# bridgedp/hunter_bipedal_control

Hardware: NVIDIA H100
Metric: MPC+WBC control-step solves/sec (Hunter N=100) (higher is better)
Workload: dtype f64

## Files before the change

hunter_bipedal_control_b200/csrc/hb_sqp.cuh:

```cuda
#pragma once
#include "hb_common.cuh"
#include "hb_mpc.cuh"
#include "hb_planner.h"
#include "hb_rbd.cuh"

namespace hb {

constexpr int LIN_F1 = 0, LIN_F2 = 22, LIN_A1 = 44, LIN_A2 = 242, LIN_BF1 = 440, LIN_BF2 = 476, LIN_BV1 = 512, LIN_BV2 = 572,
              LIN_EPOS = 632, LIN_EVEL = 644, LIN_DPQ = 656, LIN_DVX = 812, LIN_DVV = 1076, LIN_STRIDE = 1200;
constexpr int NTMAX = 16;
constexpr int NVMAX = 8;
constexpr int PJ_BT = 0, PJ_AT = 144, PJ_PXV = 342, PJ_NV = 562, PJ_BTV = 642, PJ_QV = 664, PJ_RV = 686, PJ_META = 702, PJ_PEV = 710,
              PJ_QT = 720, PJ_PT = 1204, PJ_RF = 1380, PJ_RN = 1416, PJ_STRIDE = 1480;
constexpr int PJ_RT_PACKED = PJ_STRIDE - PJ_RF;
static_assert(PJ_AT + 9 * NX == PJ_PXV && PJ_RN + NVMAX * NVMAX == PJ_STRIDE && PJ_PEV + NJ == PJ_QT, "projected record blocks are contiguous");
static_assert(PJ_QT % 2 == 0 && PJ_PT % 2 == 0 && PJ_RF % 2 == 0 && PJ_STRIDE % 2 == 0, "bulk-copied blocks start on 16 bytes");
constexpr int RK_STRIDE = NTMAX * NX + NTMAX;

struct LinHalf {
  double x[NX], u[NU], x2[NX], f[NX];
  double Acm[6 * 16], Jc[12 * 16], dp[12 * NDIR], dv[12 * NDIR];
  double Abinv[36], AbinvAj[6 * NJ], vgen[16], epos[12], evel[12], com[3];
  double sn[NDIR], cs[NDIR];
  double dh[6 * NDIR], dcom[3 * NDIR], dvb[6 * NDIR];
  double vals[2 * 6];
};
static_assert(16 * 9 <= 6 * NDIR + 3 * NDIR + 6 * NDIR, "partial sums must fit in the dh | dcom | dvb storage");

__device__ __noinline__ void lin_half(LinHalf& sh, const ChainModel& cm, const double* xs, int hl, bool act, double* rec_f, double* rec_A, double* rec_Bf,
                                      double* rec_Bv, bool want_ee, double* rec) {
  const double m = c_model.total_mass, im = 1.0 / m;
  double* part = sh.dh;
  if (hl < NDIR) { double s, c; sincos(xs[9 + hl], &s, &c); sh.sn[hl] = s; sh.cs[hl] = c; }
  __syncwarp();
  const bool euler = hl < 6;
  const int leg = (hl < 3 || (hl >= 6 && hl < 11)) ? 0 : 1;
  const int gen = euler ? 3 + (hl % 3) : hl;
  const bool with_base = hl < 3;
  const bool vlane = (hl == 0 || hl == 3);
  {
    ChainOut<double> co;
    kin_chain_f<double>(cm, leg, with_base, [&](int i) { return xs[6 + i]; }, [&](int i) { return (i == gen) ? 1.0 : 0.0; },
                        [&](int k, double& s, double& c) { s = sh.sn[k]; c = sh.cs[k]; }, co);
#pragma unroll
    for (int i = 0; i < 3; ++i) { part[hl * 9 + i] = co.P[i]; part[hl * 9 + 3 + i] = co.Lo[i]; }
    if (vlane) {
#pragma unroll
      for (int i = 0; i < 3; ++i) sh.vals[(hl / 3) * 6 + 3 + i] = co.mc[i];
    }
#pragma unroll
    for (int t = 0; t < 2; ++t) {
      const int c = leg + 2 * t;
#pragma unroll
      for (int i = 0; i < 3; ++i) {
        sh.Jc[(3 * c + i) * 16 + gen] = co.cvel[3 * t + i];
        if (!euler) sh.Jc[(3 * (c ^ 1) + i) * 16 + gen] = 0.0;
        if (vlane) sh.epos[3 * c + i] = co.cpos[3 * t + i];
      }
    }
    if (hl < 3) {
#pragma unroll
      for (int r = 0; r < 6; ++r) sh.Acm[r * 16 + hl] = (r == hl) ? m : 0.0;
#pragma unroll
// ... 41 lines not shown
  }
  if (hl >= 6) sh.vgen[hl] = sh.u[6 + hl];
  __syncwarp();
  if (hl < NJ) {
#pragma unroll
    for (int r = 0; r < 6; ++r) { double s = 0.0; for (int c = 0; c < 6; ++c) s += sh.Abinv[6 * r + c] * sh.Acm[c * 16 + 6 + hl]; sh.AbinvAj[r * NJ + hl] = s; }
  }
  {
    const int dir = gen - 3;
    ChainOut<D1> co;
    kin_chain_f<D1>(cm, leg, with_base, [&](int i) { return D1(xs[6 + i], (i == gen) ? 1.0 : 0.0); }, [&](int i) { return D1(sh.vgen[i], 0.0); },
                    [&](int k, D1& s, D1& c) { const double sv = sh.sn[k], cv = sh.cs[k]; const double on = (k == dir) ? 1.0 : 0.0; s = D1(sv, cv * on); c = D1(cv, -sv * on); },
                    co);
#pragma unroll
    for (int i = 0; i < 3; ++i) { part[hl * 9 + i] = co.P[i].d; part[hl * 9 + 3 + i] = co.Lo[i].d; part[hl * 9 + 6 + i] = co.mc[i].d; }
    if (vlane) {
#pragma unroll
      for (int i = 0; i < 3; ++i) { sh.vals[(hl / 3) * 6 + i] = co.P[i].v; sh.vals[(hl / 3) * 6 + 3 + i] = co.mc[i].v; }
    }
#pragma unroll
    for (int t = 0; t < 2; ++t) {
      const int c = leg + 2 * t;
#pragma unroll
      for (int i = 0; i < 3; ++i) {
        const int row = 3 * c + i;
        sh.dp[row * NDIR + dir] = co.cpos[3 * t + i].d;
        sh.dv[row * NDIR + dir] = co.cvel[3 * t + i].d;
        if (!euler) { sh.dp[(3 * (c ^ 1) + i) * NDIR + dir] = 0.0; sh.dv[(3 * (c ^ 1) + i) * NDIR + dir] = 0.0; }
        if (vlane) sh.evel[row] = co.cvel[3 * t + i].v;
      }
    }
  }
  __syncwarp();
  double Pd[3], Ld[3], dc[3], Pv[3], cv[3];
  if (hl < NDIR) {
    const int la = (hl < 3) ? hl : 3 + hl;
#pragma unroll
    for (int i = 0; i < 3; ++i) {
      Pd[i] = part[la * 9 + i]; Ld[i] = part[la * 9 + 3 + i]; dc[i] = part[la * 9 + 6 + i];
      if (hl < 3) { Pd[i] += part[(3 + hl) * 9 + i]; Ld[i] += part[(3 + hl) * 9 + 3 + i]; dc[i] += part[(3 + hl) * 9 + 6 + i]; }
      dc[i] *= im;
      Pv[i] = sh.vals[i] + sh.vals[6 + i];
      cv[i] = (sh.vals[3 + i] + sh.vals[9 + i]) * im;
    }
  }
  __syncwarp();
  if (hl < NDIR) {
    sh.dh[0 * NDIR + hl] = Pd[0]; sh.dh[1 * NDIR + hl] = Pd[1]; sh.dh[2 * NDIR + hl] = Pd[2];
    sh.dh[3 * NDIR + hl] = Ld[0] - ((dc[1] * Pv[2] - dc[2] * Pv[1]) + (cv[1] * Pd[2] - cv[2] * Pd[1]));
    sh.dh[4 * NDIR + hl] = Ld[1] - ((dc[2] * Pv[0] - dc[0] * Pv[2]) + (cv[2] * Pd[0] - cv[0] * Pd[2]));
    sh.dh[5 * NDIR + hl] = Ld[2] - ((dc[0] * Pv[1] - dc[1] * Pv[0]) + (cv[0] * Pd[1] - cv[1] * Pd[0]));
    sh.dcom[0 * NDIR + hl] = dc[0]; sh.dcom[1 * NDIR + hl] = dc[1]; sh.dcom[2 * NDIR + hl] = dc[2];
  }
  __syncwarp();
  if (hl < NDIR) {
#pragma unroll
    for (int r = 0; r < 6; ++r) { double s = 0.0; for (int c = 0; c < 6; ++c) s += sh.Abinv[6 * r + c] * sh.dh[c * NDIR + hl]; sh.dvb[r * NDIR + hl] = -s; }
  }
  for (int i = hl; i < NX; i += 16) {
    double val;
    if (i < 3) {
      double s = 0.0;
      for (int c = 0; c < NC; ++c) s += sh.u[3 * c + i];
      val = s * im - (i == 2 ? HB_GRAVITY : 0.0);
    } else if (i < 6) {
      const int a = i - 3, a1 = (a + 1) % 3, a2 = (a + 2) % 3;
      double s = 0.0;
      for (int c = 0; c < NC; ++c) s += (sh.epos[3 * c + a1] - sh.com[a1]) * sh.u[3 * c + a2] - (sh.epos[3 * c + a2] - sh.com[a2]) * sh.u[3 * c + a1];
      val = s * im;
    } else if (i < 12) val = sh.vgen[i - 6];
    else val = sh.u[i];
    sh.f[i] = val;
    if (act) rec_f[i] = val;
  }
  __syncwarp();
  if (!act) return;
  for (int j = hl; j < NX; j += 16) {
    double ca[9];
#pragma unroll
    for (int i = 0; i < 9; ++i) ca[i] = 0.0;
    if (j < 6) {
#pragma unroll
      for (int r = 0; r < 6; ++r) ca[3 + r] = m * sh.Abinv[6 * r + j];
    } else if (j >= 9) {
      const int k = j - 9;
      double t0 = 0.0, t1 = 0.0, t2 = 0.0;
      for (int c = 0; c < NC; ++c) {
        const double d0 = sh.dp[(3 * c) * NDIR + k] - sh.dcom[k], d1 = sh.dp[(3 * c + 1) * NDIR + k] - sh.dcom[NDIR + k], d2 = sh.dp[(3 * c + 2) * NDIR + k] - sh.dcom[2 * NDIR + k];
        const double* F = sh.u + 3 * c;
        t0 += d1 * F[2] - d2 * F[1]; t1 += d2 * F[0] - d0 * F[2]; t2 += d0 * F[1] - d1 * F[0];
      }
      ca[0] = t0 * im; ca[1] = t1 * im; ca[2] = t2 * im;
#pragma unroll
      for (int r = 0; r < 6; ++r) ca[3 + r] = sh.dvb[r * NDIR + k];
    }
#pragma unroll
    for (int i = 0; i < 9; ++i) rec_A[i * NX + j] = ca[i];
  }
  if (hl < 12) {
    const int c = hl / 3, a = hl - 3 * c;
    const double r0 = (sh.epos[3 * c] - sh.com[0]) * im, r1 = (sh.epos[3 * c + 1] - sh.com[1]) * im, r2 = (sh.epos[3 * c + 2] - sh.com[2]) * im;
    double b0 = 0.0, b1 = 0.0, b2 = 0.0;
    if (a == 0) { b1 = r2; b2 = -r1; } else if (a == 1) { b0 = -r2; b2 = r0; } else { b0 = r1; b1 = -r0; }
    rec_Bf[0 * 12 + hl] = b0; rec_Bf[1 * 12 + hl] = b1; rec_Bf[2 * 12 + hl] = b2;
  }
  if (hl < NJ) {
#pragma unroll
    for (int r = 0; r < 6; ++r) rec_Bv[r * NJ + hl] = -sh.AbinvAj[r * NJ + hl];
  }
  if (want_ee) {
    if (hl < 12) { rec[LIN_EPOS + hl] = sh.epos[hl]; rec[LIN_EVEL + hl] = sh.evel[hl]; }
    for (int t = hl; t < 29; t += 16) {
      if (t < 6) {
        for (int r = 0; r < 12; ++r) {
          double vx = 0.0;
          for (int c = 0; c < 6; ++c) vx += sh.Jc[r * 16 + c] * sh.Abinv[6 * c + t];
          rec[LIN_DVX + r * NX + t] = vx * m;
        }
      } else if (t < 19) {
        const int k = t - 6, j = 9 + k;
        for (int r = 0; r < 12; ++r) {
          double vx = sh.dv[r * NDIR + k];
          for (int c = 0; c < 6; ++c) vx += sh.Jc[r * 16 + c] * sh.dvb[c * NDIR + k];
          rec[LIN_DPQ + r * NDIR + k] = sh.dp[r * NDIR + k];
          rec[LIN_DVX + r * NX + j] = vx;
        }
      } else {
        const int jj = t - 19;
        for (int r = 0; r < 12; ++r) {
          double vu = sh.Jc[r * 16 + 6 + jj];
          for (int c = 0; c < 6; ++c) vu -= sh.Jc[r * 16 + c] * sh.AbinvAj[c * NJ + jj];
          rec[LIN_DVV + r * NJ + jj] = vu;
        }
      }
    }
    if (hl < 12) { rec[LIN_DVX + hl * NX + 6] = 0.0; rec[LIN_DVX + hl * NX + 7] = 0.0; rec[LIN_DVX + hl * NX + 8] = 0.0; }
  }
}

struct SqpArgs {
  int B, N;
  double dt;
  const double* x_ref; const double* swing; const int32_t* mode;
  double* xt; double* ut;
  double* lin;
  double* proj;
  double* rk;
  double* dxt; double* dut; double* perf; int32_t* flags;
  const double* x0;
  const double* tk; const int32_t* nn;
  InstanceView<hb_terrain> maps;
  double* sth;
};

__device__ __forceinline__ double stance_height_lane(const SqpArgs& a, int inst, int k, int lane, unsigned flm, const double* swing) {
  double h = 0.0;
  if (lane < 4) {
    const hb_terrain* m = a.maps.of(inst);
    if (m && ((flm >> lane) & 1u)) h = hbplan::map_height(m, swing[6 * lane], swing[6 * lane + 1]);
    a.sth[((size_t)inst * (a.N + 1) + k) * 4 + lane] = h;
  }
  return h;
}
__device__ __forceinline__ int sqp_nn(const SqpArgs& a, int inst) { return a.nn ? a.nn[inst] : a.N; }
__device__ __forceinline__ double sqp_dt(const SqpArgs& a, int inst, int k) {
  if (!a.tk) return a.dt;
  const double* t = a.tk + (size_t)inst * (a.N + 1) + k;
  return t[1] - t[0];
}

#ifndef HB_LIN_MINB
#define HB_LIN_MINB 6
#endif
__global__ void __launch_bounds__(64, HB_LIN_MINB) lin_kernel(SqpArgs a) {
  extern __shared__ __align__(16) unsigned char smem_raw[];
  const int warp_in_block = threadIdx.x >> 5;
  const int lane = threadIdx.x & 31, half = lane >> 4, hl = lane & 15;
  LinHalf& sh = reinterpret_cast<LinHalf*>(smem_raw)[warp_in_block * 2 + half];
  ChainModel& cm = *reinterpret_cast<ChainModel*>(smem_raw + 4 * sizeof(LinHalf));
  chain_model_load(cm, threadIdx.x, blockDim.x);
  __syncthreads();
  const int N = a.N, NP = (N + 1) >> 1;
  const long long w = (long long)blockIdx.x * (blockDim.x >> 5) + warp_in_block;
  if (w >= (long long)a.B * NP) return;
  const int inst = (int)(w / NP), pr = (int)(w - (long long)inst * NP);
  const int nn = sqp_nn(a, inst);
  if (2 * pr >= nn) return;
  const int k = 2 * pr + half;
  const bool act = k < nn;
  const int kk = act ? k : nn - 1;
  const double* xk = (kk == 0) ? a.x0 + (size_t)inst * NX : a.xt + ((size_t)inst * (N + 1) + kk) * NX;
  const double* uk = a.ut + ((size_t)inst * N + kk) * NU;
  for (int i = hl; i < NX; i += 16) { sh.x[i] = xk[i]; sh.u[i] = uk[i]; }
  __syncwarp();
  double* rec = a.lin + ((size_t)inst * N + kk) * LIN_STRIDE;
  lin_half(sh, cm, sh.x, hl, act, rec + LIN_F1, rec + LIN_A1, rec + LIN_BF1, rec + LIN_BV1, true, rec);
  const double dtk = sqp_dt(a, inst, kk);
  for (int i = hl; i < NX; i += 16) sh.x2[i] = sh.x[i] + dtk * sh.f[i];
  __syncwarp();
  lin_half(sh, cm, sh.x2, hl, act, rec + LIN_F2, rec + LIN_A2, rec + LIN_BF2, rec + LIN_BV2, false, rec);
}

}

namespace {
using namespace hb;
struct ProbeShared { LinHalf h[2]; ChainModel cm; double rec[LIN_STRIDE]; double dummy[LIN_STRIDE]; };
__global__ void __launch_bounds__(32) probe_flow_map_kernel(int B, const double* x, const double* u, double* f, double* A, double* Bm, double* ee) {
  extern __shared__ __align__(16) unsigned char smem_raw[];
  ProbeShared& ps = *reinterpret_cast<ProbeShared*>(smem_raw);
  const int inst = blockIdx.x, lane = threadIdx.x, half = lane >> 4, hl = lane & 15;
  chain_model_load(ps.cm, threadIdx.x, blockDim.x);
  LinHalf& sh = ps.h[half];
  for (int i = hl; i < NX; i += 16) { sh.x[i] = x[(size_t)inst * NX + i]; sh.u[i] = u[(size_t)inst * NU + i]; }
  __syncwarp();
  double* rec = half == 0 ? ps.rec : ps.dummy;
  lin_half(sh, ps.cm, sh.x, hl, half == 0, rec + LIN_F1, rec + LIN_A1, rec + LIN_BF1, rec + LIN_BV1, true, rec);
  __syncwarp();
  const double im = 1.0 / c_model.total_mass;
  if (lane < NX) f[(size_t)inst * NX + lane] = ps.rec[LIN_F1 + lane];
  for (int idx = lane; idx < TS; idx += 32) {
    const int i = idx / NX, j = idx - i * NX;
    double a = 0.0, b = 0.0;
    if (i >= 3 && i < 12) a = ps.rec[LIN_A1 + (i - 3) * NX + j];
    if (j < 12) {
      if (i < 3) b = (j % 3 == i) ? im : 0.0;
      else if (i < 6) b = ps.rec[LIN_BF1 + (i - 3) * 12 + j];
    } else {
      if (i >= 6 && i < 12) b = ps.rec[LIN_BV1 + (i - 6) * NJ + j - 12];
      else if (i >= 12) b = (i == j) ? 1.0 : 0.0;
    }
    A[(size_t)inst * TS + idx] = a; Bm[(size_t)inst * TS + idx] = b;
  }
  if (ee) {
    double* o = ee + (size_t)inst * (24 + 3 * 12 * NX);
    if (lane < 12) { o[lane] = ps.rec[LIN_EPOS + lane]; o[12 + lane] = ps.rec[LIN_EVEL + lane]; }
    for (int idx = lane; idx < 12 * NX; idx += 32) {
      const int r = idx / NX, j = idx - r * NX;
      double dp = 0.0;
      if (j >= 6 && j < 9) dp = (j - 6 == r % 3) ? 1.0 : 0.0;
      else if (j >= 9) dp = ps.rec[LIN_DPQ + r * NDIR + j - 9];
      o[24 + idx] = dp;
      o[24 + 12 * NX + idx] = ps.rec[LIN_DVX + idx];
      o[24 + 24 * NX + idx] = (j >= 12) ? ps.rec[LIN_DVV + r * NJ + j - 12] : 0.0;
    }
  }
}
}

namespace hb {

__device__ __forceinline__ unsigned smem_u32(const void* p) { return static_cast<unsigned>(__cvta_generic_to_shared(p)); }
__device__ __forceinline__ void mbar_init(unsigned long long* bar, unsigned count) {
  asm volatile("mbarrier.init.shared::cta.b64 [%0], %1;\n" ::"r"(smem_u32(bar)), "r"(count) : "memory");
  asm volatile("fence.mbarrier_init.release.cluster;\n" ::: "memory");
}
__device__ __forceinline__ void mbar_expect_tx(unsigned long long* bar, unsigned bytes) {
  asm volatile("mbarrier.arrive.expect_tx.shared::cta.b64 _, [%0], %1;\n" ::"r"(smem_u32(bar)), "r"(bytes) : "memory");
}
__device__ __forceinline__ void bulk_g2s(void* smem_dst, const void* gmem_src, unsigned bytes, unsigned long long* bar) {
  asm volatile("cp.async.bulk.shared::cluster.global.mbarrier::complete_tx::bytes [%0], [%1], %2, [%3];\n" ::"r"(smem_u32(smem_dst)), "l"(gmem_src), "r"(bytes),
               "r"(smem_u32(bar))
               : "memory");
}
__device__ __forceinline__ void fence_proxy_async() { asm volatile("fence.proxy.async.shared::cta;\n" ::: "memory"); }
__device__ __forceinline__ void mbar_wait(unsigned long long* bar, unsigned phase) {
  asm volatile(
      "{\n"
      ".reg .pred P1;\n"
      "LAB_WAIT:\n"
      "mbarrier.try_wait.parity.shared::cta.b64 P1, [%0], %1;\n"
      "@P1 bra DONE;\n"
      "bra LAB_WAIT;\n"
      "DONE:\n"
      "}\n" ::"r"(smem_u32(bar)),
      "r"(phase)
      : "memory");
}

struct LqShared {
  double rec[LIN_STRIDE];
  double G[NJ * 34];
  double x[NX], u[NU], swing[24];
  double q[NX], Qd[NX], r[NU], b[NX];
  double ev[12], rowg[12], dvd[NJ], RFF[36];
  unsigned long long bar;
  int rowi[12], rowa[12], piv[NJ], freev[NJ];
};
constexpr int LQ_AD = LIN_A1, LQ_BDF = LIN_A2, LQ_BDV = LIN_A2 + 108, LQ_T = LIN_EPOS, LQ_TL = 32, LQ_GL = 34, LQ_YZ = 0, LQ_GV = 256;
static_assert(LQ_BDV + 9 * NJ <= LIN_BF1, "discrete B must fit in the A2 region");
static_assert(LQ_T + NJ * LQ_TL <= LIN_STRIDE && LQ_GV + 8 * NJ <= NJ * LQ_GL, "aliased areas overflow");
static_assert((LQ_T % 2) == 0 && (sizeof(double) * LIN_STRIDE) % 16 == 0, "T is read with 128-bit loads");

__device__ __forceinline__ void lq_model(LqShared& sh, int lane, unsigned flm, int nsw, double dt, double xn_l, double xref_l, double& cost_l, double& d2_w) {
  const Model& md = c_model;
  const double im = 1.0 / md.total_mass;
  const double* A1c = sh.rec + LIN_A1; const double* A2c = sh.rec + LIN_A2;
  const double* Bf1 = sh.rec + LIN_BF1; const double* Bf2 = sh.rec + LIN_BF2;
  const double* Bv1 = sh.rec + LIN_BV1; const double* Bv2 = sh.rec + LIN_BV2;
  const double* f1 = sh.rec + LIN_F1; const double* f2 = sh.rec + LIN_F2;
  double* Ad = sh.rec + LQ_AD; double* BdF = sh.rec + LQ_BDF; double* Bdv = sh.rec + LQ_BDV;
  double bd[9];
  double d2 = 0.0;
  if (lane < NX) {
    const int j = lane;
    double c1[9];
#pragma unroll
    for (int kk = 0; kk < 9; ++kk) c1[kk] = A1c[kk * NX + j];
#pragma unroll 1
    for (int i = 0; i < 9; ++i) {
      double s = 0.0;
#pragma unroll
      for (int kk = 0; kk < 9; ++kk) s = fma(A2c[i * NX + 3 + kk], c1[kk], s);
      Ad[i * NX + j] = 0.5 * dt * (A1c[i * NX + j] + A2c[i * NX + j] + dt * s) + ((3 + i == j) ? 1.0 : 0.0);
    }
    if (j < 12) {
      const double b0 = Bf1[j], b1 = Bf1[12 + j], b2 = Bf1[24 + j];
      const int ja = j % 3;
#pragma unroll
      for (int i = 0; i < 9; ++i) {
        const double s = A2c[i * NX + 3] * b0 + A2c[i * NX + 4] * b1 + A2c[i * NX + 5] * b2 + A2c[i * NX + ja] * im;
        const double base = (i < 3) ? (Bf1[i * 12 + j] + Bf2[i * 12 + j]) : 0.0;
        bd[i] = 0.5 * dt * (base + dt * s);
      }
    } else {
      const int jj = j - 12;
      double cb[6];
#pragma unroll
      for (int kk = 0; kk < 6; ++kk) cb[kk] = Bv1[kk * NJ + jj];
#pragma unroll
      for (int i = 0; i < 9; ++i) {
        double s = A2c[i * NX + 12 + jj];
#pragma unroll
        for (int kk = 0; kk < 6; ++kk) s = fma(A2c[i * NX + 6 + kk], cb[kk], s);
        const double base = (i >= 3) ? (Bv1[(i - 3) * NJ + jj] + Bv2[(i - 3) * NJ + jj]) : 0.0;
        bd[i] = 0.5 * dt * (base + dt * s);
      }
    }
    const double bb = sh.x[lane] + 0.5 * dt * (f1[lane] + f2[lane]) - xn_l;
    sh.b[lane] = bb; d2 = bb * bb;
  }
  d2 = warp_sum(d2);
  __syncwarp();
  if (lane < NX) {
    const int j = lane;
    if (j < 12) {
#pragma unroll
      for (int i = 0; i < 9; ++i) BdF[i * 12 + j] = bd[i];
    } else {
#pragma unroll
      for (int i = 0; i < 9; ++i) Bdv[i * NJ + j - 12] = bd[i];
    }
  }
  const double* __restrict__ ltab = g_lq_lane + lane * LQ_LANE_TAB;
  const double fz = (nsw < 4) ? md.total_mass * HB_GRAVITY / (4 - nsw) : 0.0;
  double cost = 0.0;
  if (lane < NX) {
    const double d = sh.x[lane] - xref_l;
    const double Ql = ltab[0];
    sh.q[lane] = Ql * d;
    sh.Qd[lane] = Ql;
    cost += 0.5 * Ql * d * d;
    double s = 0.0;
    if (lane < 12) { double dul = sh.u[lane]; if ((lane % 3) == 2 && ((flm >> (lane / 3)) & 1u)) dul -= fz; s = ltab[1] * dul; cost += 0.5 * dul * s; }
    else {
#pragma unroll
      for (int j = 0; j < NJ; ++j) s = fma(ltab[2 + j], sh.u[12 + j], s);
      cost += 0.5 * sh.u[lane] * s;
    }
    sh.r[lane] = s;
  }
  if (lane < 12) {
// ... 27 lines not shown
      if (lane < 10) { sh.q[12 + lane] += p1; sh.Qd[12 + lane] += p2; }
      else if (lane < 20) { const int j = lane - 10; sh.r[12 + j] += p1; sh.dvd[j] = p2; }
      else if (lane < 24) { const int c = lane - 20; sh.r[3 * c + 2] += p1; sh.RFF[c * 9 + 8] += p2; }
    }
    __syncwarp();
    if (on && lane >= 24) {
      const int c = lane - 24;
      const double it = 1.0 / tn, it32 = 1.0 / (tn * t2);
      const double g0 = -Fx * it, g1 = -Fy * it, g2 = HB_FRICTION_MU;
      const double h00 = -(Fy * Fy + HB_FRICTION_REGULARIZATION) * it32, h01 = Fx * Fy * it32, h11 = -(Fx * Fx + HB_FRICTION_REGULARIZATION) * it32;
      double* Rc = sh.RFF + c * 9;
      sh.r[3 * c] += p1 * g0; sh.r[3 * c + 1] += p1 * g1; sh.r[3 * c + 2] += p1 * g2;
      Rc[0] += p2 * g0 * g0 + p1 * h00; Rc[1] += p2 * g0 * g1 + p1 * h01; Rc[2] += p2 * g0 * g2;
      Rc[3] += p2 * g1 * g0 + p1 * h01; Rc[4] += p2 * g1 * g1 + p1 * h11; Rc[5] += p2 * g1 * g2;
      Rc[6] += p2 * g2 * g0;            Rc[7] += p2 * g2 * g1;            Rc[8] += p2 * g2 * g2;
      shiftsum = -p1 * HB_FRICTION_HESSIAN_SHIFT;
    }
  }
  shiftsum = warp_sum(shiftsum);
  __syncwarp();
  if (lane < NX) sh.Qd[lane] += shiftsum;
  if (lane < 12) sh.RFF[(lane / 3) * 9 + (lane % 3) * 4] += shiftsum;
  else if (lane >= 16 && lane < 16 + NJ) sh.dvd[lane - 16] += shiftsum;
  cost_l = cost; d2_w = d2;
}

template <int NSW>
__device__ __forceinline__ void lq_node(LqShared& sh, const SqpArgs& a, int inst, int k, int lane, unsigned flm, double dt, double cost, double d2) {
  constexpr int MR = 12 - 2 * NSW, NP = 2 * NSW, NF = 3 * (4 - NSW), GL = LQ_GL, TL = LQ_TL;
  const int N = a.N;
  const Model& md = c_model;
  const double im = 1.0 / md.total_mass;
  double* out = a.proj + ((size_t)inst * N + k) * PJ_STRIDE;
  const double* epos = sh.rec + LIN_EPOS; const double* evel = sh.rec + LIN_EVEL;
  const double* dpq = sh.rec + LIN_DPQ; const double* dvx = sh.rec + LIN_DVX; const double* dvv = sh.rec + LIN_DVV;
  double* Ad = sh.rec + LQ_AD; double* BdF = sh.rec + LQ_BDF; double* Bdv = sh.rec + LQ_BDV; double* T = sh.rec + LQ_T;
  double* G = sh.G; double* YZ = sh.G + LQ_YZ; double* GV = sh.G + LQ_GV;
  if (lane == 0) {
    int mr = 0;
#pragma unroll
    for (int c = 0; c < 4; ++c) {
      if ((flm >> c) & 1u) {
#pragma unroll
        for (int ax = 0; ax < 3; ++ax) { sh.rowi[mr] = 3 * c + ax; sh.rowa[mr] = ax; sh.rowg[mr] = (ax == 2) ? (double)HB_ZEROVEL_Z_GAIN : 0.0; ++mr; }
      } else { sh.rowi[mr] = 3 * c + 2; sh.rowa[mr] = 2; sh.rowg[mr] = (double)HB_POSITION_ERROR_GAIN; ++mr; }
    }
  }
  __syncwarp();
  double hrow = 0.0;
  if (a.sth) hrow = __shfl_sync(HB_FULL_MASK, stance_height_lane(a, inst, k, lane, flm, sh.swing), lane < MR ? sh.rowi[lane] / 3 : 0);
  double e2 = 0.0;
  if (lane < MR) {
    const int row = sh.rowi[lane], c = row / 3, ax = row - 3 * c;
    double evv;
    if ((flm >> c) & 1u) {
      evv = evel[row] + (ax == 2 ? HB_ZEROVEL_Z_GAIN * epos[row] + HB_ZEROVEL_Z_OFFSET : 0.0);
      if (ax == 2 && a.sth) evv -= HB_ZEROVEL_Z_GAIN * hrow;
    } else evv = evel[row] - sh.swing[6 * c + 5] + HB_POSITION_ERROR_GAIN * (epos[row] - sh.swing[6 * c + 2]);
    sh.ev[lane] = evv;
    e2 = evv * evv;
  }
  if (lane >= 16 && lane < 28) { const int j = lane - 16; if (!((flm >> (j / 3)) & 1u)) e2 += sh.u[j] * sh.u[j]; }
  e2 = warp_sum(e2);
  {
    double xr[MR];
#pragma unroll
    for (int r = 0; r < MR; ++r) {
      const int row = sh.rowi[r];
      double v;
      if (lane < NJ) v = dvv[row * NJ + lane];
      else {
        const int jj = lane - NJ;
        double px = 0.0;
        if (jj >= 6 && jj < 9) px = (jj - 6 == sh.rowa[r]) ? 1.0 : 0.0;
        else if (jj >= 9) px = dpq[row * NDIR + jj - 9];
        v = -(dvx[row * NX + jj] + sh.rowg[r] * px);
      }
      xr[r] = v;
    }
#pragma unroll 1
    for (int i = 0; i < NJ; ++i) {
      double s = 0.0;
#pragma unroll
      for (int r = 0; r < MR; ++r) s = fma(dvv[sh.rowi[r] * NJ + i], xr[r], s);
      G[i * GL + lane] = s;
    }
    if (lane < NJ) {
      double s = 0.0;
#pragma unroll
      for (int r = 0; r < MR; ++r) s = fma(-xr[r], sh.ev[r], s);
      G[lane * GL + NJ + NX] = s;
      sh.piv[lane] = 0;
    }
  }
  __syncwarp();
  double dmax = lane < NJ ? G[lane * GL + lane] : 0.0;
  if (NSW > 0) dmax = fmax(dmax, 1.0);
  dmax = warp_max(dmax);
  const double tol = 1e-9 * fmax(dmax, 1e-300);
  for (int step = 0; step < NJ; ++step) {
    double dv = (lane < NJ && !sh.piv[lane]) ? G[lane * GL + lane] : -1.0;
    int pi = lane;
#pragma unroll
    for (int o = 8; o > 0; o >>= 1) {
      const double ov = __shfl_xor_sync(HB_FULL_MASK, dv, o);
      const int oi = __shfl_xor_sync(HB_FULL_MASK, pi, o);
      if (ov > dv || (ov == dv && oi < pi)) { dv = ov; pi = oi; }
    }
    dv = __shfl_sync(HB_FULL_MASK, dv, 0); pi = __shfl_sync(HB_FULL_MASK, pi, 0);
// ... 21 lines not shown
  if (nv > NVMAX) { nv = NVMAX; overflow = true; }
  if (NF + nv > NTMAX) { nv = NTMAX - NF; overflow = true; }
  const int nt = NF + nv;
  __syncwarp();
  const int cc = lane - NX;
  const bool nlane = cc >= 0 && cc < nv;
  double tc[NJ];
  {
    const int fc = (cc >= 0 && cc < NVMAX && cc < nv) ? sh.freev[cc] : -1;
#pragma unroll
    for (int i = 0; i < NJ; ++i) {
      const bool pv = sh.piv[i] != 0;
      double v = 0.0;
      if (lane < NX) v = pv ? G[i * GL + NJ + lane] : 0.0;
      else if (fc >= 0) v = pv ? -G[i * GL + fc] : ((i == fc) ? 1.0 : 0.0);
      else if (lane == 30) v = pv ? G[i * GL + NJ + NX] : 0.0;
      tc[i] = v;
    }
  }
  __syncwarp();
  if (NP > 0) {
    int p = 0;
#pragma unroll
    for (int c = 0; c < 4; ++c) {
      if ((flm >> c) & 1u) continue;
#pragma unroll
      for (int ax = 0; ax < 2; ++ax) {
        const int row = 3 * c + ax;
        double v = 0.0;
        if (lane < NX) {
          double px = 0.0;
          if (lane >= 6 && lane < 9) px = (lane - 6 == ax) ? 1.0 : 0.0;
          else if (lane >= 9) px = dpq[row * NDIR + lane - 9];
          v = dvx[row * NX + lane] + HB_XY_POSITION_GAIN * px;
        } else if (lane == 30) v = evel[row] - sh.swing[6 * c + 3 + ax] + HB_XY_POSITION_GAIN * (epos[row] - sh.swing[6 * c + ax]);
        if (p < NP) {
          YZ[p * TL + lane] = v;
          if (lane < NJ) GV[p * NJ + lane] = dvv[row * NJ + lane];
        }
        ++p;
      }
    }
  }
  __syncwarp();
#pragma unroll
  for (int i = 0; i < NJ; ++i) T[i * TL + lane] = tc[i];
  const double* tl = T + lane;
  double wyz[NP > 0 ? NP : 1];
  if (NP > 0) {
    if (lane < NP) { const double g = YZ[lane * TL + 30]; cost += 0.5 * HB_SOFT_SWING_WEIGHT * g * g; }
    __syncwarp();
    double yz[NP > 0 ? NP : 1];
#pragma unroll
    for (int p = 0; p < NP; ++p) yz[p] = YZ[p * TL + lane];
#pragma unroll 1
    for (int kk = 0; kk < NJ; ++kk) {
      const double t = tl[kk * TL];
#pragma unroll
      for (int p = 0; p < NP; ++p) yz[p] = fma(GV[p * NJ + kk], t, yz[p]);
    }
#pragma unroll
    for (int p = 0; p < NP; ++p) {
      wyz[p] = HB_SOFT_SWING_WEIGHT * yz[p];
      YZ[p * TL + lane] = yz[p];
    }
  }
  cost = warp_sum(cost);
// ... 16 lines not shown
      else if (nlane) out[PJ_PT + cc * NX + i] = dt * s;
    } else if (i < NX + NVMAX) {
      if (nlane && i - NX < nv) out[PJ_RN + (i - NX) * NVMAX + cc] = dt * s;
    } else {
      if (lane < NX) out[PJ_QV + lane] = dt * (sh.q[lane] + s + lin);
      else if (nlane) out[PJ_RV + NF + cc] = dt * (s + lin);
    }
  };
#pragma unroll 1
  for (int i = 0; i < 30; i += 2) {
    double s0 = 0.0, s1 = 0.0;
#pragma unroll
    for (int kk = 0; kk < NJ; ++kk) {
      const double2 t = *reinterpret_cast<const double2*>(T + kk * TL + i);
      s0 = fma(t.x, rb[kk], s0); s1 = fma(t.y, rb[kk], s1);
    }
#pragma unroll
    for (int p = 0; p < NP; ++p) {
      const double2 y = *reinterpret_cast<const double2*>(YZ + p * TL + i);
      s0 = fma(y.x, wyz[p], s0); s1 = fma(y.y, wyz[p], s1);
    }
    m_store(i, s0); m_store(i + 1, s1);
  }
  {
    double s = 0.0;
#pragma unroll
    for (int kk = 0; kk < NJ; ++kk) s = fma(T[kk * TL + 30], rb[kk], s);
#pragma unroll
    for (int p = 0; p < NP; ++p) s = fma(YZ[p * TL + 30], wyz[p], s);
    m_store(30, s);
  }
  double at9[9];
#pragma unroll
  for (int i = 0; i < 9; ++i) at9[i] = (lane < NX) ? Ad[i * NX + lane] : 0.0;
#pragma unroll 1
  for (int kk = 0; kk < NJ; ++kk) {
    const double t = tl[kk * TL];
#pragma unroll
    for (int i = 0; i < 9; ++i) at9[i] = fma(Bdv[i * NJ + kk], t, at9[i]);
  }
  if (lane == 30) {
#pragma unroll
    for (int i = 0; i < 9; ++i) sh.b[3 + i] += at9[i];
#pragma unroll
    for (int kk = 0; kk < NJ; ++kk) sh.b[12 + kk] += dt * tl[kk * TL];
  }
  const bool fcol = lane < NF;
  const int col = nlane ? NF + cc : lane;
  int sj = 0;
  if (fcol) {
    int cnt = 0;
#pragma unroll
    for (int c = 0; c < 4; ++c) if ((flm >> c) & 1u) { if (lane >= cnt && lane < cnt + 3) sj = 3 * c + lane - cnt; cnt += 3; }
  }
  if (lane < NX) {
#pragma unroll
    for (int i = 0; i < 9; ++i) out[PJ_AT + i * NX + lane] = at9[i];
#pragma unroll
    for (int i = 0; i < NJ; ++i) out[PJ_PXV + i * NX + lane] = tl[i * TL];
  } else if (nlane) {
#pragma unroll
    for (int i = 0; i < NJ; ++i) out[PJ_NV + i * NVMAX + cc] = tl[i * TL];
  } else if (lane == 30) {
#pragma unroll
    for (int i = 0; i < NJ; ++i) out[PJ_PEV + i] = tl[i * TL];
  }
  if (fcol || nlane) {
#pragma unroll
    for (int i = 0; i < 9; ++i) out[PJ_BT + i * NTMAX + col] = fcol ? BdF[i * 12 + sj] : at9[i];
  }
  if (fcol) {
    const int sa = sj % 3;
    out[PJ_RV + col] = dt * sh.r[sj];
#pragma unroll
    for (int ax = 0; ax < 3; ++ax) out[PJ_RF + 9 * (lane / 3) + ax * 3 + sa] = dt * sh.RFF[(sj / 3) * 9 + ax * 3 + sa];
  }
  __syncwarp();
  if (lane < NX) {
    const int i = lane;
    double s = sh.b[i];
    if (NSW > 0) {
#pragma unroll
      for (int c = 0; c < 4; ++c) {
        if ((flm >> c) & 1u) continue;
        if (i < 3) s -= dt * im * sh.u[3 * c + i];
        else if (i < 12) s -= BdF[(i - 3) * 12 + 3 * c] * sh.u[3 * c] + BdF[(i - 3) * 12 + 3 * c + 1] * sh.u[3 * c + 1] + BdF[(i - 3) * 12 + 3 * c + 2] * sh.u[3 * c + 2];
      }
    }
    out[PJ_BTV + lane] = s;
  }
  if (lane == 0) { out[PJ_META] = nt; out[PJ_META + 1] = NF; out[PJ_META + 2] = nv; out[PJ_META + 3] = dt * cost; out[PJ_META + 4] = dt * d2; out[PJ_META + 5] = dt * e2; out[PJ_META + 6] = overflow ? 1.0 : 0.0; out[PJ_META + 7] = dt; }
}

#ifndef HB_LQ_MINB
#define HB_LQ_MINB 15
#endif
static_assert(HB_LQ_MINB * (sizeof(LqShared) + 1024) <= 228 * 1024, "lq_kernel must fit HB_LQ_MINB blocks per SM");
__global__ void __launch_bounds__(32, HB_LQ_MINB) lq_kernel(SqpArgs a) {
  extern __shared__ __align__(16) unsigned char smem_raw[];
  LqShared& sh = *reinterpret_cast<LqShared*>(smem_raw);
  const int lane = threadIdx.x;
  const int N = a.N;
  const long long w = blockIdx.x;
  const int inst = (int)(w / N), k = (int)(w - (long long)inst * N);
  if (k >= sqp_nn(a, inst)) return;
  const double* grec = a.lin + ((size_t)inst * N + k) * LIN_STRIDE;
  const double* xk = (k == 0) ? a.x0 + (size_t)inst * NX : a.xt + ((size_t)inst * (N + 1) + k) * NX;
  if (lane == 0) {
    constexpr unsigned REC_BYTES = (LIN_DVV + 12 * NJ) * sizeof(double), V_BYTES = NX * sizeof(double), SW_BYTES = 24 * sizeof(double);
    mbar_init(&sh.bar, 1);
    mbar_expect_tx(&sh.bar, REC_BYTES + 2 * V_BYTES + SW_BYTES);
    bulk_g2s(sh.rec, grec, REC_BYTES, &sh.bar);
    bulk_g2s(sh.x, xk, V_BYTES, &sh.bar);
    bulk_g2s(sh.u, a.ut + ((size_t)inst * N + k) * NU, V_BYTES, &sh.bar);
    bulk_g2s(sh.swing, a.swing + ((size_t)inst * (N + 1) + k) * 24, SW_BYTES, &sh.bar);
  }
  __syncwarp();
  const int mode = a.mode[(size_t)inst * (N + 1) + k];
  double xn_l = 0.0, xref_l = 0.0;
  if (lane < NX) { xn_l = a.xt[((size_t)inst * (N + 1) + k + 1) * NX + lane]; xref_l = a.x_ref[((size_t)inst * (N + 1) + k) * NX + lane]; }
  int nsw = 0;
#pragma unroll
  for (int c = 0; c < 4; ++c) nsw += contact_flag(mode, c) ? 0 : 1;
  mbar_wait(&sh.bar, 0);
  const double dt = sqp_dt(a, inst, k);
  const unsigned flm = (contact_flag(mode, 0) ? 1u : 0u) | (contact_flag(mode, 1) ? 2u : 0u) | (contact_flag(mode, 2) ? 4u : 0u) | (contact_flag(mode, 3) ? 8u : 0u);
  double cost, d2;
  lq_model(sh, lane, flm, nsw, dt, xn_l, xref_l, cost, d2);
  if (nsw == 2) lq_node<2>(sh, a, inst, k, lane, flm, dt, cost, d2);
  else if (nsw == 0) lq_node<0>(sh, a, inst, k, lane, flm, dt, cost, d2);
  else lq_node<4>(sh, a, inst, k, lane, flm, dt, cost, d2);
}


template <int N, class AF>
__device__ __forceinline__ void acc_rows(double (&c)[N], AF a, const double* __restrict__ B, int ldb, int kn) {
#pragma unroll 2
  for (int k = 0; k < kn; ++k) {
    const double ak = a(k);
    const double* br = B + k * ldb;
#pragma unroll
    for (int j = 0; j < N; j += 2) {
// ... 523 lines not shown
```

Baseline: 190,500.

## Compact linearization record by storing only nonzero A/B blocks

Replaces the dense per-node linearization record (full A rows, force-arm B matrix, zero-padded contact Jacobian columns) with a compact stage layout. Only the nonzero momentum and joint blocks, COM and end-effector positions are stored, and the force-arm B is recomputed on the fly. This shrinks global writes, the bulk copy into shared memory, and the LQ shared footprint, which allows raising min blocks per SM from 15 to 16. lin_half becomes forceinline and is called from a loop. The cost is extra index logic and small recomputation in the consumers.

New measurement: 193,600, median of 6. 1.7% higher.

```diff
diff --git a/hunter_bipedal_control_b200/csrc/hb_sqp.cuh b/hunter_bipedal_control_b200/csrc/hb_sqp.cuh
--- a/hunter_bipedal_control_b200/csrc/hb_sqp.cuh
+++ b/hunter_bipedal_control_b200/csrc/hb_sqp.cuh
@@ -6,8 +6,29 @@
 
 namespace hb {
 
-constexpr int LIN_F1 = 0, LIN_F2 = 22, LIN_A1 = 44, LIN_A2 = 242, LIN_BF1 = 440, LIN_BF2 = 476, LIN_BV1 = 512, LIN_BV2 = 572,
-              LIN_EPOS = 632, LIN_EVEL = 644, LIN_DPQ = 656, LIN_DVX = 812, LIN_DVV = 1076, LIN_STRIDE = 1200;
+constexpr int LS_F = 0, LS_AM = 22, LS_AQ = 58, LS_COM = 175, LS_EPOS = 178, LS_BV = 190, LIN_STAGE = 250;
+constexpr int LIN_S1 = 0, LIN_S2 = LIN_STAGE, LIN_EVEL = 2 * LIN_STAGE, LIN_DPQ = 512, LIN_DVX = 668, LIN_DVX_LD = 19, LIN_DVV = 896,
+              LIN_STRIDE = 1016;
+static_assert(LS_AM == LS_F + NX && LS_AQ == LS_AM + 36 && LS_COM == LS_AQ + 9 * 13 && LS_EPOS == LS_COM + 3 && LS_BV == LS_EPOS + 12 &&
+              LIN_STAGE == LS_BV + 6 * NJ, "stage blocks are contiguous");
+static_assert(LIN_DPQ == LIN_EVEL + 12 && LIN_DVX == LIN_DPQ + 12 * NDIR && LIN_DVV == LIN_DVX + 12 * LIN_DVX_LD && LIN_STRIDE == LIN_DVV + 12 * NJ,
+              "contact kinematics blocks are contiguous");
+static_assert(LIN_STAGE % 2 == 0 && LIN_STRIDE % 2 == 0, "node records and their stage blocks start on 16 bytes");
+__device__ __forceinline__ double lin_a_at(const double* st, int r, int j) {
+  const double v = st[(j >= 9) ? LS_AQ + r * 13 + j - 9 : LS_AM + (r - 3) * 6 + min(j, 5)];
+  return (j >= 9 || (j < 6 && r >= 3)) ? v : 0.0;
+}
+__device__ __forceinline__ double lin_dvx_at(const double* rec, int row, int j) {
+  const double v = rec[LIN_DVX + row * LIN_DVX_LD + (j < 6 ? j : j - 3)];
+  return (j >= 6 && j < 9) ? 0.0 : v;
+}
+__device__ __forceinline__ void lin_force_arm(const double* st, int j, double im, double& b0, double& b1, double& b2) {
+  const int c = j / 3, a = j - 3 * c;
+  const double* ep = st + LS_EPOS + 3 * c; const double* cm = st + LS_COM;
+  const double r0 = __dmul_rn(ep[0] - cm[0], im), r1 = __dmul_rn(ep[1] - cm[1], im), r2 = __dmul_rn(ep[2] - cm[2], im);
+  b0 = 0.0; b1 = 0.0; b2 = 0.0;
+  if (a == 0) { b1 = r2; b2 = -r1; } else if (a == 1) { b0 = -r2; b2 = r0; } else { b0 = r1; b1 = -r0; }
+}
 constexpr int NTMAX = 16;
 constexpr int NVMAX = 8;
 constexpr int PJ_BT = 0, PJ_AT = 144, PJ_PXV = 342, PJ_NV = 562, PJ_BTV = 642, PJ_QV = 664, PJ_RV = 686, PJ_META = 702, PJ_PEV = 710,
@@ -24,11 +45,11 @@
   double sn[NDIR], cs[NDIR];
   double dh[6 * NDIR], dcom[3 * NDIR], dvb[6 * NDIR];
   double vals[2 * 6];
+  double dt;
 };
 static_assert(16 * 9 <= 6 * NDIR + 3 * NDIR + 6 * NDIR, "partial sums must fit in the dh | dcom | dvb storage");
 
-__device__ __noinline__ void lin_half(LinHalf& sh, const ChainModel& cm, const double* xs, int hl, bool act, double* rec_f, double* rec_A, double* rec_Bf,
-                                      double* rec_Bv, bool want_ee, double* rec) {
+__device__ __forceinline__ void lin_half(LinHalf& sh, const ChainModel& cm, const double* xs, int hl, bool act, double* st, bool want_ee, double* rec) {
   const double m = c_model.total_mass, im = 1.0 / m;
   double* part = sh.dh;
   if (hl < NDIR) { double s, c; sincos(xs[9 + hl], &s, &c); sh.sn[hl] = s; sh.cs[hl] = c; }
@@ -136,9 +157,10 @@
     }
   }
   __syncwarp();
-  double Pd[3], Ld[3], dc[3], Pv[3], cv[3];
-  if (hl < NDIR) {
+  double dq[9];
+  {
     const int la = (hl < 3) ? hl : 3 + hl;
+    double Pd[3], Ld[3], dc[3], Pv[3], cv[3];
 #pragma unroll
     for (int i = 0; i < 3; ++i) {
       Pd[i] = part[la * 9 + i]; Ld[i] = part[la * 9 + 3 + i]; dc[i] = part[la * 9 + 6 + i];
@@ -147,14 +169,18 @@
       Pv[i] = sh.vals[i] + sh.vals[6 + i];
       cv[i] = (sh.vals[3 + i] + sh.vals[9 + i]) * im;
     }
+    dq[0] = Pd[0]; dq[1] = Pd[1]; dq[2] = Pd[2];
+    dq[3] = Ld[0] - ((dc[1] * Pv[2] - dc[2] * Pv[1]) + (cv[1] * Pd[2] - cv[2] * Pd[1]));
+    dq[4] = Ld[1] - ((dc[2] * Pv[0] - dc[0] * Pv[2]) + (cv[2] * Pd[0] - cv[0] * Pd[2]));
+    dq[5] = Ld[2] - ((dc[0] * Pv[1] - dc[1] * Pv[0]) + (cv[0] * Pd[1] - cv[1] * Pd[0]));
+    dq[6] = dc[0]; dq[7] = dc[1]; dq[8] = dc[2];
   }
   __syncwarp();
   if (hl < NDIR) {
-    sh.dh[0 * NDIR + hl] = Pd[0]; sh.dh[1 * NDIR + hl] = Pd[1]; sh.dh[2 * NDIR + hl] = Pd[2];
-    sh.dh[3 * NDIR + hl] = Ld[0] - ((dc[1] * Pv[2] - dc[2] * Pv[1]) + (cv[1] * Pd[2] - cv[2] * Pd[1]));
-    sh.dh[4 * NDIR + hl] = Ld[1] - ((dc[2] * Pv[0] - dc[0] * Pv[2]) + (cv[2] * Pd[0] - cv[0] * Pd[2]));
-    sh.dh[5 * NDIR + hl] = Ld[2] - ((dc[0] * Pv[1] - dc[1] * Pv[0]) + (cv[0] * Pd[1] - cv[1] * Pd[0]));
-    sh.dcom[0 * NDIR + hl] = dc[0]; sh.dcom[1 * NDIR + hl] = dc[1]; sh.dcom[2 * NDIR + hl] = dc[2];
+#pragma unroll
+    for (int r = 0; r < 6; ++r) sh.dh[r * NDIR + hl] = dq[r];
+#pragma unroll
+    for (int r = 0; r < 3; ++r) sh.dcom[r * NDIR + hl] = dq[6 + r];
   }
   __syncwarp();
   if (hl < NDIR) {
@@ -175,59 +201,49 @@
     } else if (i < 12) val = sh.vgen[i - 6];
     else val = sh.u[i];
     sh.f[i] = val;
-    if (act) rec_f[i] = val;
+    if (act) st[LS_F + i] = val;
   }
   __syncwarp();
   if (!act) return;
-  for (int j = hl; j < NX; j += 16) {
-    double ca[9];
-#pragma unroll
-    for (int i = 0; i < 9; ++i) ca[i] = 0.0;
-    if (j < 6) {
-#pragma unroll
-      for (int r = 0; r < 6; ++r) ca[3 + r] = m * sh.Abinv[6 * r + j];
-    } else if (j >= 9) {
-      const int k = j - 9;
+  for (int t = hl; t < 19; t += 16) {
+    if (t < 6) {
+#pragma unroll
+      for (int r = 0; r < 6; ++r) st[LS_AM + r * 6 + t] = m * sh.Abinv[6 * r + t];
+    } else {
+      const int k = t - 6;
       double t0 = 0.0, t1 = 0.0, t2 = 0.0;
       for (int c = 0; c < NC; ++c) {
         const double d0 = sh.dp[(3 * c) * NDIR + k] - sh.dcom[k], d1 = sh.dp[(3 * c + 1) * NDIR + k] - sh.dcom[NDIR + k], d2 = sh.dp[(3 * c + 2) * NDIR + k] - sh.dcom[2 * NDIR + k];
         const double* F = sh.u + 3 * c;
         t0 += d1 * F[2] - d2 * F[1]; t1 += d2 * F[0] - d0 * F[2]; t2 += d0 * F[1] - d1 * F[0];
       }
-      ca[0] = t0 * im; ca[1] = t1 * im; ca[2] = t2 * im;
-#pragma unroll
-      for (int r = 0; r < 6; ++r) ca[3 + r] = sh.dvb[r * NDIR + k];
-    }
-#pragma unroll
-    for (int i = 0; i < 9; ++i) rec_A[i * NX + j] = ca[i];
-  }
-  if (hl < 12) {
-    const int c = hl / 3, a = hl - 3 * c;
-    const double r0 = (sh.epos[3 * c] - sh.com[0]) * im, r1 = (sh.epos[3 * c + 1] - sh.com[1]) * im, r2 = (sh.epos[3 * c + 2] - sh.com[2]) * im;
-    double b0 = 0.0, b1 = 0.0, b2 = 0.0;
-    if (a == 0) { b1 = r2; b2 = -r1; } else if (a == 1) { b0 = -r2; b2 = r0; } else { b0 = r1; b1 = -r0; }
-    rec_Bf[0 * 12 + hl] = b0; rec_Bf[1 * 12 + hl] = b1; rec_Bf[2 * 12 + hl] = b2;
-  }
+      st[LS_AQ + k] = t0 * im; st[LS_AQ + 13 + k] = t1 * im; st[LS_AQ + 26 + k] = t2 * im;
+#pragma unroll
+      for (int r = 0; r < 6; ++r) st[LS_AQ + (3 + r) * 13 + k] = sh.dvb[r * NDIR + k];
+    }
+  }
+  if (hl < 12) st[LS_EPOS + hl] = sh.epos[hl];
+  if (hl < 3) st[LS_COM + hl] = sh.com[hl];
   if (hl < NJ) {
 #pragma unroll
-    for (int r = 0; r < 6; ++r) rec_Bv[r * NJ + hl] = -sh.AbinvAj[r * NJ + hl];
+    for (int r = 0; r < 6; ++r) st[LS_BV + r * NJ + hl] = -sh.AbinvAj[r * NJ + hl];
   }
   if (want_ee) {
-    if (hl < 12) { rec[LIN_EPOS + hl] = sh.epos[hl]; rec[LIN_EVEL + hl] = sh.evel[hl]; }
+    if (hl < 12) rec[LIN_EVEL + hl] = sh.evel[hl];
     for (int t = hl; t < 29; t += 16) {
       if (t < 6) {
         for (int r = 0; r < 12; ++r) {
           double vx = 0.0;
           for (int c = 0; c < 6; ++c) vx += sh.Jc[r * 16 + c] * sh.Abinv[6 * c + t];
-          rec[LIN_DVX + r * NX + t] = vx * m;
+          rec[LIN_DVX + r * LIN_DVX_LD + t] = vx * m;
         }
       } else if (t < 19) {
-        const int k = t - 6, j = 9 + k;
+        const int k = t - 6;
         for (int r = 0; r < 12; ++r) {
           double vx = sh.dv[r * NDIR + k];
           for (int c = 0; c < 6; ++c) vx += sh.Jc[r * 16 + c] * sh.dvb[c * NDIR + k];
           rec[LIN_DPQ + r * NDIR + k] = sh.dp[r * NDIR + k];
-          rec[LIN_DVX + r * NX + j] = vx;
+          rec[LIN_DVX + r * LIN_DVX_LD + t] = vx;
         }
       } else {
         const int jj = t - 19;
@@ -238,7 +254,6 @@
         }
       }
     }
-    if (hl < 12) { rec[LIN_DVX + hl * NX + 6] = 0.0; rec[LIN_DVX + hl * NX + 7] = 0.0; rec[LIN_DVX + hl * NX + 8] = 0.0; }
   }
 }
 
@@ -296,13 +311,18 @@
   const double* xk = (kk == 0) ? a.x0 + (size_t)inst * NX : a.xt + ((size_t)inst * (N + 1) + kk) * NX;
   const double* uk = a.ut + ((size_t)inst * N + kk) * NU;
   for (int i = hl; i < NX; i += 16) { sh.x[i] = xk[i]; sh.u[i] = uk[i]; }
+  if (hl == 0) sh.dt = sqp_dt(a, inst, kk);
   __syncwarp();
   double* rec = a.lin + ((size_t)inst * N + kk) * LIN_STRIDE;
-  lin_half(sh, cm, sh.x, hl, act, rec + LIN_F1, rec + LIN_A1, rec + LIN_BF1, rec + LIN_BV1, true, rec);
-  const double dtk = sqp_dt(a, inst, kk);
-  for (int i = hl; i < NX; i += 16) sh.x2[i] = sh.x[i] + dtk * sh.f[i];
-  __syncwarp();
-  lin_half(sh, cm, sh.x2, hl, act, rec + LIN_F2, rec + LIN_A2, rec + LIN_BF2, rec + LIN_BV2, false, rec);
+#pragma unroll 1
+  for (int s = 0; s < 2; ++s) {
+    lin_half(sh, cm, s == 0 ? sh.x : sh.x2, hl, act, rec + (s == 0 ? LIN_S1 : LIN_S2), s == 0, rec);
+    if (s == 0) {
+      const double dtk = sh.dt;
+      for (int i = hl; i < NX; i += 16) sh.x2[i] = sh.x[i] + dtk * sh.f[i];
+      __syncwarp();
+    }
+  }
 }
 
 }
@@ -319,33 +339,34 @@
   for (int i = hl; i < NX; i += 16) { sh.x[i] = x[(size_t)inst * NX + i]; sh.u[i] = u[(size_t)inst * NU + i]; }
   __syncwarp();
   double* rec = half == 0 ? ps.rec : ps.dummy;
-  lin_half(sh, ps.cm, sh.x, hl, half == 0, rec + LIN_F1, rec + LIN_A1, rec + LIN_BF1, rec + LIN_BV1, true, rec);
+  lin_half(sh, ps.cm, sh.x, hl, half == 0, rec + LIN_S1, true, rec);
   __syncwarp();
   const double im = 1.0 / c_model.total_mass;
-  if (lane < NX) f[(size_t)inst * NX + lane] = ps.rec[LIN_F1 + lane];
+  const double* st = ps.rec + LIN_S1;
+  if (lane < NX) f[(size_t)inst * NX + lane] = st[LS_F + lane];
   for (int idx = lane; idx < TS; idx += 32) {
     const int i = idx / NX, j = idx - i * NX;
     double a = 0.0, b = 0.0;
-    if (i >= 3 && i < 12) a = ps.rec[LIN_A1 + (i - 3) * NX + j];
+    if (i >= 3 && i < 12) a = lin_a_at(st, i - 3, j);
     if (j < 12) {
       if (i < 3) b = (j % 3 == i) ? im : 0.0;
-      else if (i < 6) b = ps.rec[LIN_BF1 + (i - 3) * 12 + j];
+      else if (i < 6) { double b0, b1, b2; lin_force_arm(st, j, im, b0, b1, b2); b = (i == 3) ? b0 : (i == 4) ? b1 : b2; }
     } else {
-      if (i >= 6 && i < 12) b = ps.rec[LIN_BV1 + (i - 6) * NJ + j - 12];
+      if (i >= 6 && i < 12) b = st[LS_BV + (i - 6) * NJ + j - 12];
       else if (i >= 12) b = (i == j) ? 1.0 : 0.0;
     }
     A[(size_t)inst * TS + idx] = a; Bm[(size_t)inst * TS + idx] = b;
   }
   if (ee) {
     double* o = ee + (size_t)inst * (24 + 3 * 12 * NX);
-    if (lane < 12) { o[lane] = ps.rec[LIN_EPOS + lane]; o[12 + lane] = ps.rec[LIN_EVEL + lane]; }
+    if (lane < 12) { o[lane] = st[LS_EPOS + lane]; o[12 + lane] = ps.rec[LIN_EVEL + lane]; }
     for (int idx = lane; idx < 12 * NX; idx += 32) {
       const int r = idx / NX, j = idx - r * NX;
       double dp = 0.0;
       if (j >= 6 && j < 9) dp = (j - 6 == r % 3) ? 1.0 : 0.0;
       else if (j >= 9) dp = ps.rec[LIN_DPQ + r * NDIR + j - 9];
       o[24 + idx] = dp;
-      o[24 + 12 * NX + idx] = ps.rec[LIN_DVX + idx];
+      o[24 + 12 * NX + idx] = lin_dvx_at(ps.rec, r, j);
       o[24 + 24 * NX + idx] = (j >= 12) ? ps.rec[LIN_DVV + r * NJ + j - 12] : 0.0;
     }
   }
@@ -382,8 +403,9 @@
       : "memory");
 }
 
+constexpr int LQ_AD = LIN_STRIDE, LQ_BDF = LIN_S2, LQ_BDV = LIN_S2 + 108, LQ_T = LIN_EVEL, LQ_TL = 32, LQ_GL = 34, LQ_YZ = 0, LQ_GV = 256;
 struct LqShared {
-  double rec[LIN_STRIDE];
+  double rec[LQ_AD + 9 * 6];
   double G[NJ * 34];
   double x[NX], u[NU], swing[24];
   double q[NX], Qd[NX], r[NU], b[NX];
@@ -391,57 +413,70 @@
   unsigned long long bar;
   int rowi[12], rowa[12], piv[NJ], freev[NJ];
 };
-constexpr int LQ_AD = LIN_A1, LQ_BDF = LIN_A2, LQ_BDV = LIN_A2 + 108, LQ_T = LIN_EPOS, LQ_TL = 32, LQ_GL = 34, LQ_YZ = 0, LQ_GV = 256;
-static_assert(LQ_BDV + 9 * NJ <= LIN_BF1, "discrete B must fit in the A2 region");
+static_assert(LQ_BDV + 9 * NJ <= LIN_S2 + LIN_STAGE, "discrete B must fit in the stage-2 block");
+__device__ __forceinline__ double lq_ad_at(const double* rec, int i, int lane) {
+  if (lane >= 9) return (lane < NX) ? rec[LIN_S1 + LS_AQ + i * 13 + lane - 9] : 0.0;
+  if (lane < 6) return rec[LQ_AD + i * 6 + lane];
+  return (3 + i == lane) ? 1.0 : 0.0;
+}
 static_assert(LQ_T + NJ * LQ_TL <= LIN_STRIDE && LQ_GV + 8 * NJ <= NJ * LQ_GL, "aliased areas overflow");
 static_assert((LQ_T % 2) == 0 && (sizeof(double) * LIN_STRIDE) % 16 == 0, "T is read with 128-bit loads");
 
 __device__ __forceinline__ void lq_model(LqShared& sh, int lane, unsigned flm, int nsw, double dt, double xn_l, double xref_l, double& cost_l, double& d2_w) {
   const Model& md = c_model;
   const double im = 1.0 / md.total_mass;
-  const double* A1c = sh.rec + LIN_A1; const double* A2c = sh.rec + LIN_A2;
-  const double* Bf1 = sh.rec + LIN_BF1; const double* Bf2 = sh.rec + LIN_BF2;
-  const double* Bv1 = sh.rec + LIN_BV1; const double* Bv2 = sh.rec + LIN_BV2;
-  const double* f1 = sh.rec + LIN_F1; const double* f2 = sh.rec + LIN_F2;
-  double* Ad = sh.rec + LQ_AD; double* BdF = sh.rec + LQ_BDF; double* Bdv = sh.rec + LQ_BDV;
+  const double* s1 = sh.rec + LIN_S1; const double* s2 = sh.rec + LIN_S2;
+  const double* Am2 = s2 + LS_AM; const double* Aq2 = s2 + LS_AQ;
+  double* BdF = sh.rec + LQ_BDF; double* Bdv = sh.rec + LQ_BDV;
   double bd[9];
   double d2 = 0.0;
   if (lane < NX) {
     const int j = lane;
-    double c1[9];
-#pragma unroll
-    for (int kk = 0; kk < 9; ++kk) c1[kk] = A1c[kk * NX + j];
+    double c1[6];
+#pragma unroll
+    for (int kk = 0; kk < 3; ++kk) { c1[kk] = lin_a_at(s1, kk, j); c1[3 + kk] = lin_a_at(s1, 6 + kk, j); }
+    double* adc = (j >= 9) ? sh.rec + LIN_S1 + LS_AQ + j - 9 : sh.rec + LQ_AD + j;
+    const int adl = (j >= 9) ? 13 : 6;
+    const bool ads = j < 6 || j >= 9;
 #pragma unroll 1
     for (int i = 0; i < 9; ++i) {
       double s = 0.0;
-#pragma unroll
-      for (int kk = 0; kk < 9; ++kk) s = fma(A2c[i * NX + 3 + kk], c1[kk], s);
-      Ad[i * NX + j] = 0.5 * dt * (A1c[i * NX + j] + A2c[i * NX + j] + dt * s) + ((3 + i == j) ? 1.0 : 0.0);
+      if (i >= 3) {
+#pragma unroll
+        for (int kk = 0; kk < 3; ++kk) s = fma(Am2[(i - 3) * 6 + 3 + kk], c1[kk], s);
+      }
+#pragma unroll
+      for (int kk = 0; kk < 3; ++kk) s = fma(Aq2[i * 13 + kk], c1[3 + kk], s);
+      const double ad = 0.5 * dt * (lin_a_at(s1, i, j) + lin_a_at(s2, i, j) + dt * s) + ((3 + i == j) ? 1.0 : 0.0);
+      if (ads) adc[i * adl] = ad;
     }
     if (j < 12) {
-      const double b0 = Bf1[j], b1 = Bf1[12 + j], b2 = Bf1[24 + j];
+      double b0, b1, b2, e0, e1, e2;
+      lin_force_arm(s1, j, im, b0, b1, b2);
+      lin_force_arm(s2, j, im, e0, e1, e2);
       const int ja = j % 3;
 #pragma unroll
       for (int i = 0; i < 9; ++i) {
-        const double s = A2c[i * NX + 3] * b0 + A2c[i * NX + 4] * b1 + A2c[i * NX + 5] * b2 + A2c[i * NX + ja] * im;
-        const double base = (i < 3) ? (Bf1[i * 12 + j] + Bf2[i * 12 + j]) : 0.0;
+        double s = 0.0;
+        if (i >= 3) { const double* a2 = Am2 + (i - 3) * 6; s = a2[3] * b0 + a2[4] * b1 + a2[5] * b2 + a2[ja] * im; }
+        const double base = (i == 0) ? b0 + e0 : (i == 1) ? b1 + e1 : (i == 2) ? b2 + e2 : 0.0;
         bd[i] = 0.5 * dt * (base + dt * s);
       }
     } else {
       const int jj = j - 12;
-      double cb[6];
-#pragma unroll
-      for (int kk = 0; kk < 6; ++kk) cb[kk] = Bv1[kk * NJ + jj];
+      double cb[3];
+#pragma unroll
+      for (int kk = 0; kk < 3; ++kk) cb[kk] = s1[LS_BV + (3 + kk) * NJ + jj];
 #pragma unroll
       for (int i = 0; i < 9; ++i) {
-        double s = A2c[i * NX + 12 + jj];
-#pragma unroll
-        for (int kk = 0; kk < 6; ++kk) s = fma(A2c[i * NX + 6 + kk], cb[kk], s);
-        const double base = (i >= 3) ? (Bv1[(i - 3) * NJ + jj] + Bv2[(i - 3) * NJ + jj]) : 0.0;
+        double s = Aq2[i * 13 + 3 + jj];
+#pragma unroll
+        for (int kk = 0; kk < 3; ++kk) s = fma(Aq2[i * 13 + kk], cb[kk], s);
+        const double base = (i >= 3) ? (s1[LS_BV + (i - 3) * NJ + jj] + s2[LS_BV + (i - 3) * NJ + jj]) : 0.0;
         bd[i] = 0.5 * dt * (base + dt * s);
       }
     }
-    const double bb = sh.x[lane] + 0.5 * dt * (f1[lane] + f2[lane]) - xn_l;
+    const double bb = sh.x[lane] + 0.5 * dt * (s1[LS_F + lane] + s2[LS_F + lane]) - xn_l;
     sh.b[lane] = bb; d2 = bb * bb;
   }
   d2 = warp_sum(d2);
@@ -535,9 +570,9 @@
   const Model& md = c_model;
   const double im = 1.0 / md.total_mass;
   double* out = a.proj + ((size_t)inst * N + k) * PJ_STRIDE;
-  const double* epos = sh.rec + LIN_EPOS; const double* evel = sh.rec + LIN_EVEL;
-  const double* dpq = sh.rec + LIN_DPQ; const double* dvx = sh.rec + LIN_DVX; const double* dvv = sh.rec + LIN_DVV;
-  double* Ad = sh.rec + LQ_AD; double* BdF = sh.rec + LQ_BDF; double* Bdv = sh.rec + LQ_BDV; double* T = sh.rec + LQ_T;
+  const double* epos = sh.rec + LIN_S1 + LS_EPOS; const double* evel = sh.rec + LIN_EVEL;
+  const double* dpq = sh.rec + LIN_DPQ; const double* dvv = sh.rec + LIN_DVV;
+  double* BdF = sh.rec + LQ_BDF; double* Bdv = sh.rec + LQ_BDV; double* T = sh.rec + LQ_T;
   double* G = sh.G; double* YZ = sh.G + LQ_YZ; double* GV = sh.G + LQ_GV;
   if (lane == 0) {
     int mr = 0;
@@ -577,7 +612,7 @@
         double px = 0.0;
         if (jj >= 6 && jj < 9) px = (jj - 6 == sh.rowa[r]) ? 1.0 : 0.0;
         else if (jj >= 9) px = dpq[row * NDIR + jj - 9];
-        v = -(dvx[row * NX + jj] + sh.rowg[r] * px);
+        v = -(lin_dvx_at(sh.rec, row, jj) + sh.rowg[r] * px);
       }
       xr[r] = v;
     }
@@ -665,7 +700,7 @@
           double px = 0.0;
           if (lane >= 6 && lane < 9) px = (lane - 6 == ax) ? 1.0 : 0.0;
           else if (lane >= 9) px = dpq[row * NDIR + lane - 9];
-          v = dvx[row * NX + lane] + HB_XY_POSITION_GAIN * px;
+          v = lin_dvx_at(sh.rec, row, lane) + HB_XY_POSITION_GAIN * px;
         } else if (lane == 30) v = evel[row] - sh.swing[6 * c + 3 + ax] + HB_XY_POSITION_GAIN * (epos[row] - sh.swing[6 * c + ax]);
         if (p < NP) {
           YZ[p * TL + lane] = v;
@@ -748,7 +783,7 @@
   }
   double at9[9];
 #pragma unroll
-  for (int i = 0; i < 9; ++i) at9[i] = (lane < NX) ? Ad[i * NX + lane] : 0.0;
+  for (int i = 0; i < 9; ++i) at9[i] = lq_ad_at(sh.rec, i, lane);
 #pragma unroll 1
   for (int kk = 0; kk < NJ; ++kk) {
     const double t = tl[kk * TL];
@@ -809,7 +844,7 @@
 }
 
 #ifndef HB_LQ_MINB
-#define HB_LQ_MINB 15
+#define HB_LQ_MINB 16
 #endif
 static_assert(HB_LQ_MINB * (sizeof(LqShared) + 1024) <= 228 * 1024, "lq_kernel must fit HB_LQ_MINB blocks per SM");
 __global__ void __launch_bounds__(32, HB_LQ_MINB) lq_kernel(SqpArgs a) {
@@ -823,7 +858,7 @@
   const double* grec = a.lin + ((size_t)inst * N + k) * LIN_STRIDE;
   const double* xk = (k == 0) ? a.x0 + (size_t)inst * NX : a.xt + ((size_t)inst * (N + 1) + k) * NX;
   if (lane == 0) {
-    constexpr unsigned REC_BYTES = (LIN_DVV + 12 * NJ) * sizeof(double), V_BYTES = NX * sizeof(double), SW_BYTES = 24 * sizeof(double);
+    constexpr unsigned REC_BYTES = LIN_STRIDE * sizeof(double), V_BYTES = NX * sizeof(double), SW_BYTES = 24 * sizeof(double);
     mbar_init(&sh.bar, 1);
     mbar_expect_tx(&sh.bar, REC_BYTES + 2 * V_BYTES + SW_BYTES);
     bulk_g2s(sh.rec, grec, REC_BYTES, &sh.bar);
```
